# bioinfo-pf-curie/mpiBWA

Hardware: AMD Instinct MI355X
Metric: Mreads/s (whole node) 2x150 bp PE vs GRCh38-size reference; SAM bit-match (higher is better)
Workload: dtype int32

## Files before the change

mpibwa_amd/csrc/chain_kernel.hip:

```cpp
#include <hip/hip_runtime.h>
#include <hipcub/hipcub.hpp>
#include <cstdlib>
#include <mutex>
#include <utility>
#include <vector>
#include "hip_util.h"
#include "device.h"
#include "sortutil.h"

namespace mbw {

namespace {

typedef long long i64;

#define CK_MAXCH 9
#define CK_MAXCH_SMALL 4
#define CK_MAXSEEDS_SMALL 16
#define CK_MAXSEEDS 64
#define CK_MAXSEEDS_BIG 255
enum { F_POS_LO = 0, F_POS_HI, F_FIRST_Q, F_LAST_R_LO, F_LAST_R_HI, F_LAST_Q, F_LAST_LEN, F_RID, F_N, F_W, F_KEPT, F_FIRSTOV, F_NFIELDS };

template <int MAXCH>
struct StoreLds {
// ... 258 lines not shown
{
	extern __shared__ uint32_t lds_raw[];
	StoreLds<MAXCH> L;
	L.lane = threadIdx.x;
	L.tab = lds_raw;
	L.cid_ = (uint8_t *)(lds_raw + F_NFIELDS * MAXCH * 64);
	L.ord_ = L.cid_ + (MAXS + 1) * 64;
	L.tmp_ = L.ord_ + 16 * 64;
	int rd = blockIdx.x * 64 + threadIdx.x;
	if (list) { if (rd >= (int)*list_n) return; rd = list[rd]; }
	if (rd >= n_reads) return;
	const int ns = n_seeds[rd], lq = lens[rd];
	const int *gap = tab, *noflt = tab + 5 * tab_stride;
	if (LO >= 0) { if (n_chains[rd] != -1 || ns <= LO) return; }
	else if (ns == 0) { n_chains[rd] = 0; return; }
	if (ns > MAXS || !noflt[lq]) { n_chains[rd] = -1; return; }
	n_chains[rd] = chain_read(L, P, rd, ns, lq, seed_off[rd], l_rep, sa, qbl, ann_off, ann_alt, n_seqs, gap, chains, seeds, srt);
}

__global__ void __launch_bounds__(256)
chain_pick_kernel(int n_reads, const int *__restrict__ lens, const int *__restrict__ n_seeds, const int *__restrict__ n_chains,
                  const int *__restrict__ noflt, int lo, int hi, int cap, int *__restrict__ list, unsigned int *__restrict__ count)
{
	const int rd = blockIdx.x * 256 + threadIdx.x;
	const bool mine = rd < n_reads && n_chains[rd] == -1 && n_seeds[rd] > lo && n_seeds[rd] <= hi && noflt[lens[rd]] != 0;
	const unsigned long long m = __ballot(mine);
	if (!m) return;
	const int lane = threadIdx.x & 63, lead = __ffsll((long long)m) - 1;
	unsigned int base = 0;
	if (lane == lead) base = atomicAdd(count, (unsigned int)__popcll(m));
	base = __shfl(base, lead);
	const unsigned int at = base + (unsigned int)__popcll(m & ((1ull << lane) - 1));
	if (mine && at < (unsigned int)cap) list[at] = rd;
}

#define HV_NONE 0xFFFFu
__host__ __device__ constexpr size_t hv_lds_bytes(int cap) { return (size_t)(cap + 64) * 24; }
__host__ __device__ constexpr size_t hv_scratch_bytes(int cap) { return (size_t)cap * (4 + 7 * 2 + 8 + 4) + 512; }
struct HvStore {
	uint32_t *rid;
	uint16_t *head, *cid, *next, *ord;
	uint32_t *last_off;
	uint16_t *first_q, *last_q, *last_len, *tail, *nmem;
};
__device__ __forceinline__ bool hv_lt(uint32_t a, uint32_t b) { return (a >> 16) > (b >> 16); }
#define HV_FRAMES 32
__device__ __forceinline__ void hv_sort(uint32_t *a, int n)
{
	int fs[HV_FRAMES], ft[HV_FRAMES], fd[HV_FRAMES];
	ks_introsort_at(n, [a](int k) -> uint32_t & { return a[k]; }, KsFramesAt{fs, ft, fd}, hv_lt);
}
__device__ __forceinline__ void hv_sync()
{
	__builtin_amdgcn_fence(__ATOMIC_RELEASE, "wavefront");
	__builtin_amdgcn_wave_barrier();
	__builtin_amdgcn_fence(__ATOMIC_ACQUIRE, "wavefront");
}
__device__ __forceinline__ int hv_bcast(int v) { return __builtin_amdgcn_readfirstlane(v); }

template <int CAP>
__global__ void __launch_bounds__(64)
chain_heavy_kernel(ChainParams P, const int *__restrict__ list, const unsigned int *__restrict__ list_n, unsigned int *work, int list_cap,
                   const int *__restrict__ lens, const int *__restrict__ n_seeds, const int *__restrict__ l_rep, const i64 *__restrict__ seed_off,
                   const unsigned long long *__restrict__ sa, const int32_t *__restrict__ qbl, const i64 *__restrict__ ann_off,
                   const uint8_t *__restrict__ ann_alt, int n_seqs, const int *__restrict__ gap, uint8_t *__restrict__ scratch,
                   DevChain *__restrict__ chains, DevSeed *__restrict__ seeds, unsigned int *__restrict__ srt, int *__restrict__ n_chains)
// ... 339 lines not shown
	std::lock_guard<std::mutex> lk(side_mu);
	for (auto &e : sides) if (e.first == st) return e.second;
	ChainSide sd;
	for (int k = 0; k < 2; ++k) { HIP_OK(hipStreamCreateWithFlags(&sd.s[k], hipStreamNonBlocking)); HIP_OK(hipEventCreateWithFlags(&sd.join[k], hipEventDisableTiming)); }
	HIP_OK(hipEventCreateWithFlags(&sd.fork, hipEventDisableTiming));
	sides.emplace_back(st, sd);
	return sd;
}

void launch_chain(void *stream, const ChainParams &P, int n_reads, const int *d_len, const int *d_nseeds, const int *d_lrep,
                  const int64_t *d_seed_off, const uint64_t *d_sa, const int32_t *d_qbl, const int64_t *d_ann_off, const uint8_t *d_ann_alt,
                  int n_seqs, const int *d_tab, int tab_stride, DevChain *d_chains, DevSeed *d_seeds, unsigned int *d_srt, int *d_nchains,
                  void *d_scratch)
{
	if (n_reads <= 0) return;
	const size_t lds_s = chain_lds_bytes(CK_MAXSEEDS_SMALL, CK_MAXCH_SMALL), lds = chain_lds_bytes(CK_MAXSEEDS, CK_MAXCH), lds_big = chain_lds_bytes(CK_MAXSEEDS_BIG, CK_MAXCH);
	static bool s_attr = false;
	if (!s_attr) {
		if (lds > 64 * 1024) HIP_OK(hipFuncSetAttribute((const void *)chain_kernel<CK_MAXSEEDS, CK_MAXCH, 0>, hipFuncAttributeMaxDynamicSharedMemorySize, (int)lds));
		if (lds_big > 64 * 1024) HIP_OK(hipFuncSetAttribute((const void *)chain_kernel<CK_MAXSEEDS_BIG, CK_MAXCH, CK_MAXSEEDS>, hipFuncAttributeMaxDynamicSharedMemorySize, (int)lds_big));
		s_attr = true;
	}
	hipStream_t st = (hipStream_t)stream;
	const dim3 grid((n_reads + 63) / 64), block(64);
#define CHAIN_ARGS P, n_reads, d_len, d_nseeds, d_lrep, (const i64 *)d_seed_off, (const unsigned long long *)d_sa, d_qbl, (const i64 *)d_ann_off, d_ann_alt, n_seqs, d_tab, \
	               tab_stride, d_chains, d_seeds, d_srt, d_nchains
#define LAUNCH_HEAVY(CAP, waves, s, list, n, work, scr)                                                                                                       \
	hipLaunchKernelGGL((chain_heavy_kernel<CAP>), dim3(waves), dim3(64), hv_lds_bytes(CAP), s, P, (const int *)(list), (const unsigned int *)(n), work,      \
	                   n_reads, d_len, d_nseeds, d_lrep, (const i64 *)d_seed_off, (const unsigned long long *)d_sa, d_qbl, (const i64 *)d_ann_off, d_ann_alt, \
	                   n_seqs, d_tab, scr, d_chains, d_seeds, d_srt, d_nchains)
	const int big = getenv("MPIBWA_CHAIN_BIG") ? atoi(getenv("MPIBWA_CHAIN_BIG")) : 2;
	int *list_a = (int *)d_scratch, *list_b = list_a + n_reads;
	unsigned int *count = (unsigned int *)(list_b + n_reads);
	int *list_h1 = (int *)((uint8_t *)count + 512), *list_h2 = list_h1 + n_reads;
	uint8_t *scr_t = (uint8_t *)(((uintptr_t)(list_h2 + n_reads) + 255) & ~(uintptr_t)255);
	uint8_t *scr_s = scr_t + HV_WAVES_T * hv_scratch_bytes(256), *scr_l = scr_s + HV_WAVES_S * hv_scratch_bytes(1024);
	HIP_OK(hipMemsetAsync(count, 0, 64, st));
	auto pick = [&](int lo, int hi, int *list, unsigned int *n) {
		hipLaunchKernelGGL(chain_pick_kernel, dim3((n_reads + 255) / 256), dim3(256), 0, st, n_reads, d_len, d_nseeds, (const int *)d_nchains, d_tab + 5 * tab_stride, lo, hi,
		                   n_reads, list, n);
	};
	hipLaunchKernelGGL((chain_kernel<CK_MAXSEEDS_SMALL, CK_MAXCH_SMALL, -1>), grid, block, lds_s, st, CHAIN_ARGS, (const int *)nullptr, (const unsigned int *)nullptr);
	pick(0, CK_MAXSEEDS, list_a, count + 1);
	hipLaunchKernelGGL((chain_kernel<CK_MAXSEEDS, CK_MAXCH, 0>), grid, block, lds, st, CHAIN_ARGS, (const int *)list_a, (const unsigned int *)(count + 1));
	if (big >= 1) {
		pick(CK_MAXSEEDS, CK_MAXSEEDS_BIG, list_b, count + 2);
		hipLaunchKernelGGL((chain_kernel<CK_MAXSEEDS_BIG, CK_MAXCH, CK_MAXSEEDS>), grid, block, lds_big, st, CHAIN_ARGS, (const int *)list_b, (const unsigned int *)(count + 2));
	}
	if (big >= 2) {
		int *list_t = list_a;
		pick(0, CK_MAXSEEDS_BIG, list_t, count);
		const bool heavy = !(getenv("MPIBWA_CHAIN_HEAVY") && atoi(getenv("MPIBWA_CHAIN_HEAVY")) == 0);
		ChainSide sd = {};
		if (heavy) {
			static bool s_attr2 = false;
			if (!s_attr2) {
				HIP_OK(hipFuncSetAttribute((const void *)chain_heavy_kernel<4096>, hipFuncAttributeMaxDynamicSharedMemorySize, (int)hv_lds_bytes(4096)));
				s_attr2 = true;
			}
			pick(CK_MAXSEEDS_BIG, 1024, list_h1, count + 4);
			pick(1024, 4096, list_h2, count + 6);
			sd = chain_side_streams(st);
			HIP_OK(hipEventRecord(sd.fork, st));
			for (int k = 0; k < 2; ++k) HIP_OK(hipStreamWaitEvent(sd.s[k], sd.fork, 0));
			LAUNCH_HEAVY(4096, HV_WAVES_L, sd.s[0], list_h2, count + 6, count + 7, scr_l);
			LAUNCH_HEAVY(1024, HV_WAVES_S, sd.s[1], list_h1, count + 4, count + 5, scr_s);
		}
		LAUNCH_HEAVY(256, HV_WAVES_T, st, list_t, count, count + 3, scr_t);
		if (heavy)
			for (int k = 0; k < 2; ++k) { HIP_OK(hipEventRecord(sd.join[k], sd.s[k])); HIP_OK(hipStreamWaitEvent(st, sd.join[k], 0)); }
	}
#undef LAUNCH_HEAVY
#undef CHAIN_ARGS
	HIP_OK(hipGetLastError());
}

}
```

mpibwa_amd/csrc/phase1.hip:

```cpp
#include "pipeline.h"

namespace mbw {

static int c2a_early_mode() { const char *e = getenv("MPIBWA_C2A_EARLY"); return e ? atoi(e) : 1; }
static bool dev_dedup_on()
{
	const char *on = getenv("MPIBWA_DEV_DEDUP"), *off = getenv("MPIBWA_HOST_DEDUP");
	return on && atoi(on) != 0 && !(off && atoi(off) != 0);
}
class TurnLock {
public:
	void lock()
	{
		std::unique_lock<std::mutex> lk(m_);
		const unsigned long long mine = next_++;
		cv_.wait(lk, [&]() { return serving_ == mine; });
	}
	void unlock()
	{
		{ std::lock_guard<std::mutex> lk(m_); ++serving_; }
		cv_.notify_all();
	}
private:
	std::mutex m_;
	std::condition_variable cv_;
	unsigned long long next_ = 0, serving_ = 0;
};
static TurnLock g_smem_turn, g_c2a_turn;
static std::mutex g_pes_lock;

void Call::phase1(int lo, int hi, LaneBufs &L, HostBuf &reg_arena, hipStream_t lst, int lane_thr, P1 &ps)
{
	static const bool take_turns = !(getenv("MPIBWA_TURNS") && atoi(getenv("MPIBWA_TURNS")) == 0);
	const int n_sb = hi - lo;
	bseq1_t *seqs_r = seqs + lo;
	const int64_t *d_off_r = D.d_off + lo;
	const int *d_len_r = D.d_len + lo;
	const uint8_t *d_seq = D.d_seq;
	HIP_OK(hipSetDevice(ix.device));
	stage(2);
	parallel_for(lane_thr, n_sb, 4096, [&](int i) {
		char *s = seqs_r[i].seq;
		uint8_t *d = flat + off[lo + i];
		for (int k = 0; k < seqs_r[i].l_seq; ++k) {
			s[k] = s[k] < 4 ? s[k] : (char)nt4_table[(uint8_t)s[k]];
			d[k] = (uint8_t)s[k];
		}
	});
	HIP_OK(hipMemcpyAsync((uint8_t *)W.seq.p + off[lo], flat + off[lo], (size_t)(off[hi] - off[lo]) + (hi == n ? 16 : 0), hipMemcpyHostToDevice, lst));
	EvTimer ev_smem, ev_sa, ev_ext;
	unsigned long long *d_cnt = (unsigned long long *)L.cnt.ensure(256);
	unsigned long long *cnt = (unsigned long long *)L.h_cnt.ensure(256);
	const int TS = max_len + 2;
	std::vector<int> tab;
	c2a_length_tables(opt, max_len, tab);
	const int *gap_h = tab.data();
	int *d_tab = (int *)L.tab.ensure(tab.size() * 4);
	HIP_OK(hipMemcpyAsync(d_tab, tab.data(), tab.size() * 4, hipMemcpyHostToDevice, lst));

	double t1 = now_ms();
	uint64_t range_bases = 0;
	for (int i = 0; i < n_sb; ++i) range_bases += lens[lo + i];
	int cap = std::max(64, std::min(max_len, 96));
	uint64_t *d_intv; int *d_nintv;
	size_t per_quad = 0;
	int n_quads = smem_grid_quads(max_len, &per_quad);
	void *d_scr = L.scratch.ensure(per_quad * n_quads);
	int *d_nseeds = (int *)L.nseeds.ensure((size_t)n_sb * 4), *d_lrep = (int *)L.lrep.ensure((size_t)n_sb * 4);
	int *nseeds = (int *)L.h_nseeds.ensure((size_t)n_sb * 4 + 8), *lrep = (int *)L.h_lrep.ensure((size_t)n_sb * 4 + 8);
	int *nintv = (int *)L.h_nintv.ensure((size_t)n_sb * 4 + 8);
	const char *ce = getenv("MPIBWA_SMEM_COUNT");
	const bool count_blocks = ce && atoi(ce) != 0;
	for (;;) {
		d_intv = (uint64_t *)L.intv.ensure((size_t)n_sb * cap * 32);
		d_nintv = (int *)L.nintv.ensure((size_t)n_sb * 4);
		HIP_OK(hipMemsetAsync(d_cnt, 0, 256, lst));
		stage(20);
		std::unique_lock<TurnLock> turn(g_smem_turn, std::defer_lock);
		if (take_turns) turn.lock();
		stage(21);
		ev_smem.start(lst);
		launch_smem(lst, ix.fm, smem_params(opt), n_sb, d_seq, d_off_r, d_len_r, cap, d_intv, d_nintv, max_len, d_cnt, d_scr, per_quad, n_quads, count_blocks);
		ev_smem.stop(lst);
		launch_seed_prep(lst, n_sb, cap, d_intv, d_nintv, opt->max_occ, d_nseeds, d_lrep);
		HIP_OK(hipMemcpyAsync(cnt, d_cnt, 64, hipMemcpyDeviceToHost, lst));
		HIP_OK(hipMemcpyAsync(nseeds, d_nseeds, (size_t)n_sb * 4, hipMemcpyDeviceToHost, lst));
		HIP_OK(hipMemcpyAsync(lrep, d_lrep, (size_t)n_sb * 4, hipMemcpyDeviceToHost, lst));
		HIP_OK(hipMemcpyAsync(nintv, d_nintv, (size_t)n_sb * 4, hipMemcpyDeviceToHost, lst));
		stream_wait(lst);
		HIP_OK(hipGetLastError());
		if (take_turns) turn.unlock();
		ps.k_smem += ev_smem.ms();
		if (cnt[2] == 0) break;
		cap *= 4;
	}
	ps.smem_bytes = count_blocks ? cnt[1] * 64 + range_bases : 0;
	ps.smem_tab_bytes = cnt[4] * 64;
	double t2 = now_ms();
	stage(3);

	int64_t *seed_off = (int64_t *)L.h_seed_off.ensure((size_t)(n_sb + 1) * 8 + 64);
	seed_off[0] = 0;
	uint64_t n_intv = 0;
	for (int i = 0; i < n_sb; ++i) { seed_off[i + 1] = seed_off[i] + nseeds[i]; n_intv += nintv[i]; }
	const int64_t S = seed_off[n_sb];
	if (count_blocks) ps.smem_bytes += n_intv * 32;
	ps.n_intv = n_intv; ps.n_seeds = S;
	uint64_t *sa = (uint64_t *)L.h_sa.ensure((size_t)S * 8 + 8);
	int32_t *qbl = (int32_t *)L.h_qbl.ensure((size_t)S * 8 + 8);
	const bool host_chain_all = getenv("MPIBWA_HOST_CHAIN") != nullptr;
	const bool dev_chain = !host_chain_all && S > 0;
	int *nch = nullptr;
	DevChain *d_chains = nullptr; DevSeed *d_seeds = nullptr; unsigned int *d_srt = nullptr;
	if (S > 0) {
		int64_t *d_seed_off = (int64_t *)L.seed_off.ensure((size_t)(n_sb + 1) * 8);
		uint64_t *d_rows = (uint64_t *)L.rows.ensure((size_t)S * 8), *d_sa = (uint64_t *)L.sa.ensure((size_t)S * 8);
		int32_t *d_qbl = (int32_t *)L.qbl.ensure((size_t)S * 8);
		HIP_OK(hipMemcpyAsync(d_seed_off, seed_off, (size_t)(n_sb + 1) * 8, hipMemcpyHostToDevice, lst));
		launch_seed_enum(lst, n_sb, cap, d_intv, d_nintv, opt->max_occ, d_seed_off, d_rows, d_qbl);
		if (S > 0x7fffffff) die("too many seeds in one batch");
		HIP_OK(hipMemsetAsync(d_cnt, 0, 256, lst));
		ev_sa.start(lst);
		if (ix.fm.sa_full) launch_sa_dense(lst, ix.fm, (int)S, d_rows, d_sa);
		else launch_sa(lst, ix.fm, (int)S, d_rows, d_sa, d_cnt);
		ev_sa.stop(lst);
// ... 166 lines not shown
	const bool dev_dedup = dev_dedup_on();
	const uint8_t *dd_status = nullptr;
	const int *dd_m = nullptr, *dd_keep = nullptr;
	if (n_slots == 0) {
		memset(nregs, 0, (size_t)n_sb * 4);
		if (d_pr_nfirst) { HIP_OK(hipMemsetAsync(d_pr_nfirst + lo, 0, (size_t)n_sb * 4, lst)); stream_wait(lst); }
	} else {
		int *d_chain_beg = (int *)L.chain_off.ensure((size_t)n_sb * 4), *d_chain_cnt = (int *)L.chain_cnt.ensure((size_t)n_sb * 4);
		int *d_reg_beg = (int *)L.reg_off.ensure((size_t)n_sb * 4);
		d_chains = (DevChain *)L.chains.ensure((size_t)std::max<int64_t>(base + NC, 1) * sizeof(DevChain));
		d_seeds = (DevSeed *)L.seeds.ensure((size_t)n_slots * sizeof(DevSeed));
		d_srt = (unsigned int *)L.srt.ensure((size_t)n_slots * 4);
		DevReg *d_regs = (DevReg *)L.regs.ensure((size_t)n_slots * sizeof(DevReg));
		int *d_nregs = (int *)L.nregs.ensure((size_t)(n_sb + 1) * 4);
		HIP_OK(hipMemcpyAsync(d_chain_beg, chain_beg, (size_t)n_sb * 4, hipMemcpyHostToDevice, lst));
		HIP_OK(hipMemcpyAsync(d_chain_cnt, chain_cnt, (size_t)n_sb * 4, hipMemcpyHostToDevice, lst));
		HIP_OK(hipMemcpyAsync(d_reg_beg, reg_beg, (size_t)n_sb * 4, hipMemcpyHostToDevice, lst));
		if (NC) HIP_OK(hipMemcpyAsync(d_chains + base, hchains, (size_t)NC * sizeof(DevChain), hipMemcpyHostToDevice, lst));
		if (NS) HIP_OK(hipMemcpyAsync(d_seeds + base, hseeds, (size_t)NS * sizeof(DevSeed), hipMemcpyHostToDevice, lst));
		if (NS) HIP_OK(hipMemcpyAsync(d_srt + base, hsrt, (size_t)NS * 4, hipMemcpyHostToDevice, lst));
		unsigned long long *d_c2a_stat = (unsigned long long *)L.c2a_stat.ensure(C2A_STAT_SLOTS * 64);
		HIP_OK(hipMemsetAsync(d_c2a_stat, 0, C2A_STAT_SLOTS * 64, lst));
		int *order = (int *)L.h_order.ensure((size_t)n_sb * 4 + 8);
		c2a_launch_order(n_sb, nseeds, order);
		int *d_order = (int *)L.order.ensure((size_t)n_sb * 4);
		HIP_OK(hipMemcpyAsync(d_order, order, (size_t)n_sb * 4, hipMemcpyHostToDevice, lst));
		static const int heavy_t = getenv("MPIBWA_C2A_HEAVY") ? atoi(getenv("MPIBWA_C2A_HEAVY")) : 8;
		const C2aUnits units = c2a_prepare_units(lst, L.grp, heavy_t, n_sb, chain_cnt, (size_t)std::max<int64_t>(base + NC, 1), d_chain_beg, d_reg_beg,
		                                         d_chains, d_nregs, [](void *s) { stream_wait((hipStream_t)s); });
		C2aParams cp;
		ExtParams ep;
		c2a_params(opt, bns->l_pac, c2a_early_mode(), cp, ep);
		const int64_t guess = std::min<int64_t>(n_slots, (int64_t)2 * n_sb + 1024);
		uint8_t *d_dd_status = nullptr, *h_dd_status = nullptr;
		int *d_dd_m = nullptr, *d_dd_keep = nullptr, *d_dd_list = nullptr, *h_dd_m = nullptr, *h_dd_keep = nullptr;
		std::unique_ptr<EvTimer> ev_dd;
		if (dev_dedup) {
			ev_dd.reset(new EvTimer());
			d_dd_status = (uint8_t *)L.dd_status.ensure((size_t)n_sb);
			d_dd_m = (int *)L.dd_m.ensure((size_t)n_sb * 4);
			d_dd_keep = (int *)L.dd_keep.ensure((size_t)n_slots * 4);
			d_dd_list = (int *)L.dd_list.ensure(dedup_list_ints(n_sb) * 4);
			h_dd_status = (uint8_t *)L.h_dd_status.ensure((size_t)n_sb + 8);
			h_dd_m = (int *)L.h_dd_m.ensure((size_t)n_sb * 4 + 8);
			h_dd_keep = (int *)L.h_dd_keep.ensure((size_t)guess * 4 + 8);
		}
		stage(50);
		std::unique_lock<TurnLock> turn(g_c2a_turn, std::defer_lock);
		if (take_turns) turn.lock();
		stage(51);
		ev_ext.start(lst);
		launch_c2a(lst, cp, ep, n_sb, d_seq, d_off_r, d_len_r, d_chain_beg, d_chain_cnt, d_chains, d_seeds, d_srt, d_reg_beg, d_regs, d_nregs,
		           d_tab, TS, (const uint8_t *)ix.d_pac, d_c2a_stat, max_len, d_order, units.max_units > 0 ? &units : nullptr);
		ev_ext.stop(lst);
		int *d_reg_pos = (int *)L.reg_pos.ensure((size_t)(n_sb + 1) * 4);
		DevReg *d_packed = (DevReg *)L.regs_packed.ensure((size_t)n_slots * sizeof(DevReg));
		const size_t tmp_bytes = reg_pack_tmp_bytes(n_sb);
		void *d_tmp = L.pack_tmp.ensure(tmp_bytes);
		launch_reg_pack(lst, n_sb, d_reg_beg, d_nregs, d_reg_pos, d_regs, d_packed, d_tmp, tmp_bytes, units.max_units > 0 ? &units : nullptr, d_chain_beg, d_chain_cnt);
		if (d_pr_first) launch_first_reg(lst, n_sb, d_reg_pos, d_nregs, d_packed, d_pr_first + (size_t)lo * PR_MAXREG, d_pr_nfirst + lo);
		if (dev_dedup) {
			ev_dd->start(lst);
			launch_dedup(lst, dedup_params(opt, bns->l_pac), n_sb, d_packed, d_reg_pos, d_nregs, d_dd_status, d_dd_m, d_dd_keep, d_dd_list);
			ev_dd->stop(lst);
		}
		hregs = (DevReg *)L.h_regs.ensure((size_t)guess * sizeof(DevReg) + 8);
		unsigned long long *stat_h = (unsigned long long *)L.h_c2a_stat.ensure(C2A_STAT_SLOTS * 64);
		HIP_OK(hipMemcpyAsync(stat_h, d_c2a_stat, C2A_STAT_SLOTS * 64, hipMemcpyDeviceToHost, lst));
		HIP_OK(hipMemcpyAsync(nregs, d_nregs, (size_t)n_sb * 4, hipMemcpyDeviceToHost, lst));
		HIP_OK(hipMemcpyAsync(hregs, d_packed, (size_t)guess * sizeof(DevReg), hipMemcpyDeviceToHost, lst));
		if (dev_dedup) {
			HIP_OK(hipMemcpyAsync(h_dd_status, d_dd_status, (size_t)n_sb, hipMemcpyDeviceToHost, lst));
			HIP_OK(hipMemcpyAsync(h_dd_m, d_dd_m, (size_t)n_sb * 4, hipMemcpyDeviceToHost, lst));
			HIP_OK(hipMemcpyAsync(h_dd_keep, d_dd_keep, (size_t)guess * 4, hipMemcpyDeviceToHost, lst));
		}
		stream_wait(lst);
		HIP_OK(hipGetLastError());
		if (take_turns) turn.unlock();
		ps.k_ext = ev_ext.ms();
		for (int k = 0; k < 4; ++k) { cnt[k] = 0; for (int sl = 0; sl < C2A_STAT_SLOTS; ++sl) cnt[k] += stat_h[sl * 8 + k]; }
		ps.cells = cnt[0]; ps.n_ext = cnt[1];
		if (cp.early == 2 && cnt[3]) die("c2a_kernel: %llu of %llu extensions change when their row loops stop early", cnt[3], cnt[1]);
		if (getenv("MPIBWA_CPUSEC")) fprintf(stderr, "[c2a] %llu extensions, %llu without DP, %llu cells, kernel %.2f ms\n", cnt[1], cnt[2], cnt[0], ev_ext.ms());
		for (int i = 0; i < n_sb; ++i) reg_pos[i + 1] = reg_pos[i] + nregs[i];
		const int64_t NR = reg_pos[n_sb];
		if (NR > guess) {
			DevReg *all = (DevReg *)L.h_regs2.ensure((size_t)NR * sizeof(DevReg) + 8);
			HIP_OK(hipMemcpyAsync(all, d_packed, (size_t)NR * sizeof(DevReg), hipMemcpyDeviceToHost, lst));
			if (dev_dedup) {
				int *all_keep = (int *)L.h_dd_keep2.ensure((size_t)NR * 4 + 8);
				HIP_OK(hipMemcpyAsync(all_keep, d_dd_keep, (size_t)NR * 4, hipMemcpyDeviceToHost, lst));
				h_dd_keep = all_keep;
			}
			stream_wait(lst);
			hregs = all;
		}
		if (dev_dedup) {
			dd_status = h_dd_status; dd_m = h_dd_m; dd_keep = h_dd_keep;
			ps.k_dedup = ev_dd->ms();
			if (getenv("MPIBWA_CPUSEC")) {
				unsigned long long c[5] = {0, 0, 0, 0, 0};
				for (int i = 0; i < n_sb; ++i) ++c[dd_status[i] < 5 ? dd_status[i] : 0];
				fprintf(stderr, "[dedup] kernels %.2f ms; reads taken %llu, more than %d regions %llu, to patch %llu\n", ps.k_dedup, c[DD_TAKEN], DD_MAXREG,
				        c[DD_HOST_MAXREG], c[DD_HOST_PATCH]);
			}
		}
	}
	double t5 = now_ms();
	stage(6);

	const int SLACK = 4;
	std::vector<int64_t> slice(n_sb + 1);
	slice[0] = 0;
	for (int i = 0; i < n_sb; ++i) slice[i + 1] = slice[i] + nregs[i] + SLACK;
	HReg *arena = (HReg *)reg_arena.ensure((size_t)slice[n_sb] * sizeof(HReg));
	parallel_for(lane_thr, n_sb, 256, [&](int i) {
// ... 92 lines not shown
```

mpibwa_amd/csrc/pipeline.h:

```cpp
#ifndef MBW_PIPELINE_H
#define MBW_PIPELINE_H
#include <hip/hip_runtime.h>
#include <algorithm>
#include <atomic>
#include <memory>
#include <mutex>
#include <chrono>
#include <condition_variable>
#include <deque>
#include <cmath>
#include <cstdio>
#include <cstdlib>
#include <cstring>
#include <thread>
#include <vector>
#include <sys/resource.h>
#include <sys/time.h>
#include <unistd.h>

#include "hip_util.h"
#include "device.h"
#include "host.h"
#include "hprof.h"

// ... 111 lines not shown
		std::atomic<int> next{0};
		int n, nb, chunk;
		F *f;
		void work(int tid)
		{
			for (;;) {
				int b = next.fetch_add(1);
				if (b >= nb) break;
				(*f)(tid, b, b * chunk, std::min(n, (b + 1) * chunk));
			}
		}
	} R;
	R.n = n; R.nb = nb; R.chunk = chunk; R.f = &f;
	HelperPool &P = HelperPool::get();
	if (P.enabled() && n_threads > 1) {
		HelperPool::Job job;
		job.run = [](void *r, int tid) { ((Region *)r)->work(tid); };
		job.region = &R;
		P.run(n_threads - 1, job, [](void *r) { ((Region *)r)->work(0); }, &R);
		return;
	}
	std::vector<std::thread> th;
	for (int t = 1; t < n_threads; ++t) th.emplace_back([&R, t]() { R.work(t); });
	R.work(0);
	for (auto &t : th) t.join();
}

double now_ms();
double sys_sec();
long page_faults();
double cpu_sec();
void stage(int id);
void stream_wait(hipStream_t st);

struct EvTimer {
	hipEvent_t a, b;
	EvTimer() { HIP_OK(hipEventCreate(&a)); HIP_OK(hipEventCreate(&b)); }
	~EvTimer() { (void)hipEventDestroy(a); (void)hipEventDestroy(b); }
	void start(hipStream_t s) { HIP_OK(hipEventRecord(a, s)); }
	void stop(hipStream_t s) { HIP_OK(hipEventRecord(b, s)); }
	double ms() { HIP_OK(hipEventSynchronize(b)); float m = 0; HIP_OK(hipEventElapsedTime(&m, a, b)); return m; }
};

struct HostBuf {
	void *p = nullptr; size_t cap = 0;
	void *ensure(size_t bytes) { if (bytes > cap) { free(p); cap = bytes + bytes / 4 + 4096; p = malloc(cap); if (!p) die("out of memory"); } return p; }
};

struct LaneBufs {
	PinBuf h_nch, h_cbeg, h_ccnt, h_rbeg, h_nseeds, h_lrep, h_nintv, h_cnt, h_seed_off, h_c2a_stat, h_order;
	PinBuf h_sa, h_qbl, h_chains, h_seeds, h_srt, h_regs, h_regs2, h_nregs;
	DevBuf nch, chain_cnt, reg_pos, regs_packed, pack_tmp, order, chain_scratch, c2a_stat;
	C2aGroupBufs grp;
	DevBuf intv, nintv, cnt, scratch, nseeds, lrep, seed_off, rows, qbl, sa;
	DevBuf chain_off, chains, seeds, srt, reg_off, regs, nregs, tab;
	DevBuf dd_status, dd_m, dd_keep, dd_list;
	PinBuf h_dd_status, h_dd_m, h_dd_keep, h_dd_keep2;
};
struct JobBufs {
	DevBuf req, hdr, pool, cnt, lists, base, arena, used, ooff, olen;
	PinBuf h_hdr, h_pool, h_base, h_arena, h_ooff, h_olen;
};
struct ChunkBufs {
	PinBuf h_off, h_len, h_flat;
	DevBuf seq, off, len, ann_off, ann_alt, agap;
	DevBuf sdesc, squal, snames, snoff, sann_names, sann_noff;
	PinBuf h_sdesc, h_names, h_noff, h_qual;
	DevBuf pr_first, pr_nfirst, pr_ok, pr_status, pr_ptab, pr_req, pr_desc;
	PinBuf h_pr_ok, h_pr_status, h_pr_tab;
	PinBuf h_mreq[2], h_mres[2], h_mlist[2];
	DevBuf mreq[2], mres[2], mrows[2], mlist[2], mtail[2];
	PinBuf h_wwork[2], h_wlists[2], h_wloff[2], h_wmfirst[2], h_wtags[2], h_wtoff[2], h_wstatus[2];
	DevBuf wwork[2], wlists[2], wloff[2], wmfirst[2], wtags[2], wtoff[2], wstatus[2], wreq[2], wdesc[2];
	JobBufs wave_job[2];
	PinBuf h_wxcnt[2], h_wxdst[2];
	DevBuf wxreq[2], wxcnt[2], wxdst[2], xa_req[2], xa_desc;
	JobBufs xa_job[2];
	PinBuf h_areq[2];
	JobBufs host_job[2];
	JobBufs dev_job[2];
	PinBuf h_small[2];
};
static const int MAX_LANES = 4;
static const int MAX_CALLS = 12;
struct CallCtx {
	std::vector<DevBuf *> bufs;
	struct Open { Open(std::vector<DevBuf *> *l) { g_devbuf_owner = l; } } open_{&bufs};
	LaneBufs ws[MAX_LANES];
	HostBuf reg_arena[17];
	ChunkBufs gws;
	hipStream_t p_streams[MAX_LANES] = {nullptr}, a_streams[2] = {nullptr, nullptr}, d_streams[2] = {nullptr, nullptr};
	bool busy = false;
	const bseq1_t *seq_lo = nullptr, *seq_hi = nullptr;
	int calls_done = 0;
	struct Close { Close() { g_devbuf_owner = nullptr; } } close_;
	size_t device_bytes() const { size_t b = 0; for (const DevBuf *d : bufs) b += d->cap; return b; }
	void release_device() { for (DevBuf *d : bufs) d->release(); calls_done = 0; }
};

struct P1 { double k_smem = 0, k_sa = 0, k_ext = 0, k_dedup = 0, smem = 0, sa = 0, chain = 0, ext = 0, regs = 0; uint64_t smem_bytes = 0, smem_tab_bytes = 0, sa_bytes = 0, cells = 0, n_ext = 0, n_intv = 0, n_seeds = 0, n_chains = 0, n_dedup_dev = 0, n_dedup_host = 0; };

struct Job {
	JobBufs *B = nullptr;
	bool launched = false, sam_launched = false;
	hipStream_t st = 0;
	size_t n_req = 0, pool_bytes = 0, arena_bytes = 0;
	int n_reads = 0;
	AlnHdr *d_hdr = nullptr; uint8_t *d_pool = nullptr; unsigned long long *d_cnt = nullptr;
	unsigned long long *small_cnt = nullptr, *small_used = nullptr;
	EvTimer ev;
	const AlnHdrH *hdr = nullptr; const uint8_t *pool = nullptr;
	const uint8_t *sarena = nullptr; const unsigned long long *sooff = nullptr; const int *solen = nullptr;
};
struct Part {
	int lo = 0, hi = 0, slot = 0;
	AlnReqH *req = nullptr;
	size_t n_req = 0;
	std::vector<uint32_t> base;
	Job host;
	Job dev;
	MswReqH *mreq = nullptr; MswResH *mres = nullptr;
	std::vector<uint32_t> mbase;
	size_t n_mreq = 0;
	hipStream_t mst = 0;
	EvTimer mev;
	bool m_launched = false, msw_launched = false;
	std::vector<int> work;
	std::vector<unsigned> w_mfirst;
	std::vector<int> w_toff;
	std::vector<int16_t> w_tags;
	const uint8_t *wstatus = nullptr;
	int n_wave_dec = 0;
	Job wave;
// ... 101 lines not shown
```

mpibwa_amd/csrc/pipeline.hip:

```cpp
#include "pipeline.h"

namespace mbw {

static mi355x_stats_t g_stats;

static int usable_cpus_now()
{
	int hw = (int)std::thread::hardware_concurrency();
	if (hw <= 0) hw = 1;
	if (FILE *fp = fopen("/sys/fs/cgroup/cpu.max", "r")) {
		char q[64];
		long long period = 0;
		if (fscanf(fp, "%63s %lld", q, &period) == 2 && strcmp(q, "max") != 0 && period > 0) {
			long long quota = atoll(q);
			int c = (int)((quota + period - 1) / period);
			if (c >= 1 && c < hw) hw = c;
		}
		fclose(fp);
	}
	return hw;
}
int usable_cpus() { static const int c = usable_cpus_now(); return c; }

static int env_int(const char *const *names, int dflt)
// ... 62 lines not shown
	{
		while (!stop.load()) {
			int nw = 0, nh = 0, st[SAMPLE_SLOTS], ns = 0;
			for (int i = 0; i < SAMPLE_SLOTS; ++i) {
				const int v = g_stage[i].load(std::memory_order_relaxed);
				if (!v) continue;
				st[ns++] = v;
				const int id = v & 63, w = (v & STG_WAIT) != 0;
				if (w) ++nw; else if (id != 20 && id != 50) ++nh;
			}
			if (ns >= min_calls) {
				++n_samples; ++by_wait[nw]; ++by_host[nh];
				for (int k = 0; k < ns; ++k) ++in_stage[st[k] & 63][(st[k] & STG_WAIT) != 0];
				if (!nw) { ++n_gpu_idle; for (int k = 0; k < ns; ++k) ++host_when_idle[st[k] & 63]; }
				if (!nh) ++n_host_idle;
			}
			usleep(250);
		}
	}
	void report()
	{
		if (!n_samples) return;
		fprintf(stderr, "[sample] %llu samples with a call in flight; no call waiting for the GPU in %.1f %%, no call on the host in %.1f %%\n",
		        (unsigned long long)n_samples, 100.0 * n_gpu_idle / n_samples, 100.0 * n_host_idle / n_samples);
		fprintf(stderr, "[sample] calls waiting for the GPU:");
		for (int k = 0; k <= 12; ++k) fprintf(stderr, " %d:%.1f%%", k, 100.0 * by_wait[k] / n_samples);
		fprintf(stderr, "\n[sample] calls working on the host:");
		for (int k = 0; k <= 12; ++k) fprintf(stderr, " %d:%.1f%%", k, 100.0 * by_host[k] / n_samples);
		fprintf(stderr, "\n[sample] stage: mean calls in it on the host / waiting for the GPU / on the host while no call waits for the GPU\n");
		for (int id = 0; id < SAMPLE_STAGES; ++id)
			if (in_stage[id][0] + in_stage[id][1])
				fprintf(stderr, "[sample]   %2d: %.3f %.3f %.3f\n", id, (double)in_stage[id][0] / n_samples, (double)in_stage[id][1] / n_samples,
				        n_gpu_idle ? (double)host_when_idle[id] / n_gpu_idle : 0.0);
	}
};
static StageSampler *g_sampler = nullptr;
void sampler_report()
{
	if (!g_sampler) return;
	g_sampler->stop.store(true);
	g_sampler->th.join();
	g_sampler->report();
	delete g_sampler;
	g_sampler = nullptr;
}

void stream_wait(hipStream_t st)
{
	static const bool spin = getenv("MPIBWA_SPIN_WAIT") != nullptr;
	struct Mark {
		Mark() { if (t_stage) t_stage->fetch_or(STG_WAIT, std::memory_order_relaxed); }
		~Mark() { if (t_stage) t_stage->fetch_and(~STG_WAIT, std::memory_order_relaxed); }
	} mark;
	if (!spin) {
		for (;;) {
			hipError_t e = hipStreamQuery(st);
			if (e == hipSuccess) break;
			if (e != hipErrorNotReady) HIP_OK(e);
			(void)hipGetLastError();
			usleep(60);
		}
	}
	HIP_OK(hipStreamSynchronize(st));
}


void Call::pack()
{
	stage(29);
	off = (int64_t *)W.h_off.ensure((size_t)(n + 1) * 8 + 64);
	lens = (int *)W.h_len.ensure((size_t)n * 4 + 64);
	{
		const int BLK = 8192, nb = (n + BLK - 1) / BLK;
		std::vector<int64_t> bsum(nb + 1, 0);
		std::vector<int> bmax(nb, 0);
		parallel_for(n_thr, nb, 1, [&](int b) {
			const int lo = b * BLK, hi = std::min(n, lo + BLK);
			int64_t sl = 0;
			int m = 0;
			for (int i = lo; i < hi; ++i) {
				const int l = seqs[i].l_seq;
				lens[i] = l; sl += (l + 15) & ~15; m = std::max(m, l);
			}
			bsum[b + 1] = sl; bmax[b] = m;
		});
		for (int b = 0; b < nb; ++b) { bsum[b + 1] += bsum[b]; max_len = std::max(max_len, bmax[b]); }
		parallel_for(n_thr, nb, 1, [&](int b) {
			const int lo = b * BLK, hi = std::min(n, lo + BLK);
			int64_t o = bsum[b];
			for (int i = lo; i < hi; ++i) { off[i] = o; o += (lens[i] + 15) & ~15; }
		});
		off[n] = bsum[nb];
	}
	stage(30);
	flat_bytes = (size_t)off[n] + 16;
	flat = (uint8_t *)W.h_flat.ensure(flat_bytes);
// ... 322 lines not shown
```

Baseline: 6.847.

## Release GPU turn locks after kernel finishes instead of after copy-back

The seeding and extension turn locks now release once the main kernel's stop event completes, so the follow-on prep kernels, packing and device-to-host copies run outside the serialized section and the next caller can launch sooner. The turn lock is rewritten as a ticket lock with a configurable admission width, and turn queue, hold and tail clocks are recorded for diagnostics. Some buffer allocations are hoisted out of the locked region. An opt-in, size-ordered bucketing of heavy chain read lists is also added. Releasing earlier lets calls overlap on the GPU, at the cost of contention between a call's tail work and the next call's kernel.

```diff
diff --git a/mpibwa_amd/csrc/chain_kernel.hip b/mpibwa_amd/csrc/chain_kernel.hip
--- a/mpibwa_amd/csrc/chain_kernel.hip
+++ b/mpibwa_amd/csrc/chain_kernel.hip
@@ -314,6 +314,42 @@
 	base = __shfl(base, lead);
 	const unsigned int at = base + (unsigned int)__popcll(m & ((1ull << lane) - 1));
 	if (mine && at < (unsigned int)cap) list[at] = rd;
+}
+
+#define HV_BUCKETS 8
+__device__ __forceinline__ int hv_list_bucket(int ns, int &bucket, int buckets)
+{
+	if (ns <= CK_MAXSEEDS_BIG || ns > 4096) return -1;
+	const int l = ns > 1024, lo = l ? 1024 : CK_MAXSEEDS_BIG, hi = l ? 4096 : 1024;
+	bucket = buckets - 1 - (int)((long long)(ns - lo - 1) * buckets / (hi - lo));
+	return l;
+}
+__global__ void __launch_bounds__(256)
+chain_bucket_count_kernel(int n_reads, const int *__restrict__ lens, const int *__restrict__ n_seeds, const int *__restrict__ n_chains,
+                          const int *__restrict__ noflt, int buckets, unsigned int *__restrict__ cnt, unsigned int *__restrict__ n1, unsigned int *__restrict__ n2)
+{
+	const int rd = blockIdx.x * 256 + threadIdx.x;
+	if (rd >= n_reads || n_chains[rd] != -1 || noflt[lens[rd]] == 0) return;
+	int b = 0;
+	const int l = hv_list_bucket(n_seeds[rd], b, buckets);
+	if (l < 0) return;
+	atomicAdd(cnt + l * HV_BUCKETS + b, 1u);
+	atomicAdd(l ? n2 : n1, 1u);
+}
+__global__ void __launch_bounds__(256)
+chain_bucket_place_kernel(int n_reads, const int *__restrict__ lens, const int *__restrict__ n_seeds, const int *__restrict__ n_chains,
+                          const int *__restrict__ noflt, int buckets, const unsigned int *__restrict__ cnt, unsigned int *__restrict__ fill,
+                          int *__restrict__ list1, int *__restrict__ list2)
+{
+	const int rd = blockIdx.x * 256 + threadIdx.x;
+	if (rd >= n_reads || n_chains[rd] != -1 || noflt[lens[rd]] == 0) return;
+	int b = 0;
+	const int l = hv_list_bucket(n_seeds[rd], b, buckets);
+	if (l < 0) return;
+	unsigned int at = 0;
+	for (int k = 0; k < b; ++k) at += cnt[l * HV_BUCKETS + k];
+	at += atomicAdd(fill + l * HV_BUCKETS + b, 1u);
+	if (at < (unsigned int)n_reads) (l ? list2 : list1)[at] = rd;
 }
 
 #define HV_NONE 0xFFFFu
@@ -719,10 +755,11 @@
 	const int big = getenv("MPIBWA_CHAIN_BIG") ? atoi(getenv("MPIBWA_CHAIN_BIG")) : 2;
 	int *list_a = (int *)d_scratch, *list_b = list_a + n_reads;
 	unsigned int *count = (unsigned int *)(list_b + n_reads);
+	unsigned int *bucket_cnt = count + 16, *bucket_fill = bucket_cnt + 2 * HV_BUCKETS;
 	int *list_h1 = (int *)((uint8_t *)count + 512), *list_h2 = list_h1 + n_reads;
 	uint8_t *scr_t = (uint8_t *)(((uintptr_t)(list_h2 + n_reads) + 255) & ~(uintptr_t)255);
 	uint8_t *scr_s = scr_t + HV_WAVES_T * hv_scratch_bytes(256), *scr_l = scr_s + HV_WAVES_S * hv_scratch_bytes(1024);
-	HIP_OK(hipMemsetAsync(count, 0, 64, st));
+	HIP_OK(hipMemsetAsync(count, 0, (16 + 4 * HV_BUCKETS) * 4, st));
 	auto pick = [&](int lo, int hi, int *list, unsigned int *n) {
 		hipLaunchKernelGGL(chain_pick_kernel, dim3((n_reads + 255) / 256), dim3(256), 0, st, n_reads, d_len, d_nseeds, (const int *)d_nchains, d_tab + 5 * tab_stride, lo, hi,
 		                   n_reads, list, n);
@@ -745,8 +782,17 @@
 				HIP_OK(hipFuncSetAttribute((const void *)chain_heavy_kernel<4096>, hipFuncAttributeMaxDynamicSharedMemorySize, (int)hv_lds_bytes(4096)));
 				s_attr2 = true;
 			}
-			pick(CK_MAXSEEDS_BIG, 1024, list_h1, count + 4);
-			pick(1024, 4096, list_h2, count + 6);
+			const bool ordered = getenv("MPIBWA_CHAIN_ORDER") && atoi(getenv("MPIBWA_CHAIN_ORDER")) != 0;
+			const int buckets = HV_BUCKETS;
+			if (!ordered) {
+				pick(CK_MAXSEEDS_BIG, 1024, list_h1, count + 4);
+				pick(1024, 4096, list_h2, count + 6);
+			} else {
+			hipLaunchKernelGGL(chain_bucket_count_kernel, dim3((n_reads + 255) / 256), dim3(256), 0, st, n_reads, d_len, d_nseeds, (const int *)d_nchains, d_tab + 5 * tab_stride,
+			                   buckets, bucket_cnt, count + 4, count + 6);
+			hipLaunchKernelGGL(chain_bucket_place_kernel, dim3((n_reads + 255) / 256), dim3(256), 0, st, n_reads, d_len, d_nseeds, (const int *)d_nchains, d_tab + 5 * tab_stride,
+			                   buckets, (const unsigned int *)bucket_cnt, bucket_fill, list_h1, list_h2);
+			}
 			sd = chain_side_streams(st);
 			HIP_OK(hipEventRecord(sd.fork, st));
 			for (int k = 0; k < 2; ++k) HIP_OK(hipStreamWaitEvent(sd.s[k], sd.fork, 0));
diff --git a/mpibwa_amd/csrc/phase1.hip b/mpibwa_amd/csrc/phase1.hip
--- a/mpibwa_amd/csrc/phase1.hip
+++ b/mpibwa_amd/csrc/phase1.hip
@@ -1,4 +1,5 @@
 #include "pipeline.h"
+#include "turn_lock.h"
 
 namespace mbw {
 
@@ -8,30 +9,30 @@
 	const char *on = getenv("MPIBWA_DEV_DEDUP"), *off = getenv("MPIBWA_HOST_DEDUP");
 	return on && atoi(on) != 0 && !(off && atoi(off) != 0);
 }
-class TurnLock {
-public:
-	void lock()
-	{
-		std::unique_lock<std::mutex> lk(m_);
-		const unsigned long long mine = next_++;
-		cv_.wait(lk, [&]() { return serving_ == mine; });
-	}
-	void unlock()
-	{
-		{ std::lock_guard<std::mutex> lk(m_); ++serving_; }
-		cv_.notify_all();
-	}
-private:
-	std::mutex m_;
-	std::condition_variable cv_;
-	unsigned long long next_ = 0, serving_ = 0;
+static bool take_turns_on() { const char *e = getenv("MPIBWA_TURNS"); return !(e && atoi(e) == 0); }
+static bool tail_in_turn_on() { const char *e = getenv("MPIBWA_TURN_TAIL"); return e && atoi(e) != 0; }
+static const int TURN_WIDTH_SMEM = 1, TURN_WIDTH_C2A = 1;
+static void turn_widths(int &w_smem, int &w_c2a)
+{
+	w_smem = TURN_WIDTH_SMEM; w_c2a = TURN_WIDTH_C2A;
+	const char *e = getenv("MPIBWA_TURN_WIDTH");
+	if (!e || !*e) return;
+	w_smem = w_c2a = std::max(1, atoi(e));
+	if (const char *c = strchr(e, ',')) w_c2a = std::max(1, atoi(c + 1));
+}
+struct Event {
+	hipEvent_t e;
+	Event() { HIP_OK(hipEventCreate(&e)); }
+	~Event() { (void)hipEventDestroy(e); }
 };
 static TurnLock g_smem_turn, g_c2a_turn;
 static std::mutex g_pes_lock;
 
 void Call::phase1(int lo, int hi, LaneBufs &L, HostBuf &reg_arena, hipStream_t lst, int lane_thr, P1 &ps)
 {
-	static const bool take_turns = !(getenv("MPIBWA_TURNS") && atoi(getenv("MPIBWA_TURNS")) == 0);
+	const bool take_turns = take_turns_on(), tail_in_turn = tail_in_turn_on();
+	int w_smem = 1, w_c2a = 1;
+	turn_widths(w_smem, w_c2a);
 	const int n_sb = hi - lo;
 	bseq1_t *seqs_r = seqs + lo;
 	const int64_t *d_off_r = D.d_off + lo;
@@ -49,6 +50,7 @@
 	});
 	HIP_OK(hipMemcpyAsync((uint8_t *)W.seq.p + off[lo], flat + off[lo], (size_t)(off[hi] - off[lo]) + (hi == n ? 16 : 0), hipMemcpyHostToDevice, lst));
 	EvTimer ev_smem, ev_sa, ev_ext;
+	Event ev_tail;
 	unsigned long long *d_cnt = (unsigned long long *)L.cnt.ensure(256);
 	unsigned long long *cnt = (unsigned long long *)L.h_cnt.ensure(256);
 	const int TS = max_len + 2;
@@ -76,21 +78,29 @@
 		d_nintv = (int *)L.nintv.ensure((size_t)n_sb * 4);
 		HIP_OK(hipMemsetAsync(d_cnt, 0, 256, lst));
 		stage(20);
-		std::unique_lock<TurnLock> turn(g_smem_turn, std::defer_lock);
-		if (take_turns) turn.lock();
+		const double q0 = now_ms();
+		TurnHold turn(g_smem_turn, take_turns, w_smem);
+		const double q1 = now_ms();
+		double q2 = q1;
 		stage(21);
 		ev_smem.start(lst);
 		launch_smem(lst, ix.fm, smem_params(opt), n_sb, d_seq, d_off_r, d_len_r, cap, d_intv, d_nintv, max_len, d_cnt, d_scr, per_quad, n_quads, count_blocks);
 		ev_smem.stop(lst);
+		if (!tail_in_turn) { event_wait(ev_smem.b); HIP_OK(hipGetLastError()); turn.release(); q2 = now_ms(); stage(26); }
 		launch_seed_prep(lst, n_sb, cap, d_intv, d_nintv, opt->max_occ, d_nseeds, d_lrep);
 		HIP_OK(hipMemcpyAsync(cnt, d_cnt, 64, hipMemcpyDeviceToHost, lst));
 		HIP_OK(hipMemcpyAsync(nseeds, d_nseeds, (size_t)n_sb * 4, hipMemcpyDeviceToHost, lst));
 		HIP_OK(hipMemcpyAsync(lrep, d_lrep, (size_t)n_sb * 4, hipMemcpyDeviceToHost, lst));
 		HIP_OK(hipMemcpyAsync(nintv, d_nintv, (size_t)n_sb * 4, hipMemcpyDeviceToHost, lst));
+		HIP_OK(hipEventRecord(ev_tail.e, lst));
 		stream_wait(lst);
 		HIP_OK(hipGetLastError());
-		if (take_turns) turn.unlock();
-		ps.k_smem += ev_smem.ms();
+		if (tail_in_turn) { turn.release(); q2 = now_ms(); }
+		const double k_ms = ev_smem.ms();
+		float tail_ms = 0;
+		HIP_OK(hipEventElapsedTime(&tail_ms, ev_smem.b, ev_tail.e));
+		ps.k_smem += k_ms;
+		ps.tc_smem.queue += q1 - q0; ps.tc_smem.hold += q2 - q1; ps.tc_smem.kernel += k_ms; ps.tc_smem.tail += tail_ms; ++ps.tc_smem.n;
 		if (cnt[2] == 0) break;
 		cap *= 4;
 	}
@@ -323,6 +333,12 @@
 		ExtParams ep;
 		c2a_params(opt, bns->l_pac, c2a_early_mode(), cp, ep);
 		const int64_t guess = std::min<int64_t>(n_slots, (int64_t)2 * n_sb + 1024);
+		int *d_reg_pos = (int *)L.reg_pos.ensure((size_t)(n_sb + 1) * 4);
+		DevReg *d_packed = (DevReg *)L.regs_packed.ensure((size_t)n_slots * sizeof(DevReg));
+		const size_t tmp_bytes = reg_pack_tmp_bytes(n_sb);
+		void *d_tmp = L.pack_tmp.ensure(tmp_bytes);
+		hregs = (DevReg *)L.h_regs.ensure((size_t)guess * sizeof(DevReg) + 8);
+		unsigned long long *stat_h = (unsigned long long *)L.h_c2a_stat.ensure(C2A_STAT_SLOTS * 64);
 		uint8_t *d_dd_status = nullptr, *h_dd_status = nullptr;
 		int *d_dd_m = nullptr, *d_dd_keep = nullptr, *d_dd_list = nullptr, *h_dd_m = nullptr, *h_dd_keep = nullptr;
 		std::unique_ptr<EvTimer> ev_dd;
@@ -337,17 +353,16 @@
 			h_dd_keep = (int *)L.h_dd_keep.ensure((size_t)guess * 4 + 8);
 		}
 		stage(50);
-		std::unique_lock<TurnLock> turn(g_c2a_turn, std::defer_lock);
-		if (take_turns) turn.lock();
+		const double q0 = now_ms();
+		TurnHold turn(g_c2a_turn, take_turns, w_c2a);
+		const double q1 = now_ms();
+		double q2 = q1;
 		stage(51);
 		ev_ext.start(lst);
 		launch_c2a(lst, cp, ep, n_sb, d_seq, d_off_r, d_len_r, d_chain_beg, d_chain_cnt, d_chains, d_seeds, d_srt, d_reg_beg, d_regs, d_nregs,
 		           d_tab, TS, (const uint8_t *)ix.d_pac, d_c2a_stat, max_len, d_order, units.max_units > 0 ? &units : nullptr);
 		ev_ext.stop(lst);
-		int *d_reg_pos = (int *)L.reg_pos.ensure((size_t)(n_sb + 1) * 4);
-		DevReg *d_packed = (DevReg *)L.regs_packed.ensure((size_t)n_slots * sizeof(DevReg));
-		const size_t tmp_bytes = reg_pack_tmp_bytes(n_sb);
-		void *d_tmp = L.pack_tmp.ensure(tmp_bytes);
+		if (!tail_in_turn) { event_wait(ev_ext.b); HIP_OK(hipGetLastError()); turn.release(); q2 = now_ms(); stage(52); }
 		launch_reg_pack(lst, n_sb, d_reg_beg, d_nregs, d_reg_pos, d_regs, d_packed, d_tmp, tmp_bytes, units.max_units > 0 ? &units : nullptr, d_chain_beg, d_chain_cnt);
 		if (d_pr_first) launch_first_reg(lst, n_sb, d_reg_pos, d_nregs, d_packed, d_pr_first + (size_t)lo * PR_MAXREG, d_pr_nfirst + lo);
 		if (dev_dedup) {
@@ -355,8 +370,6 @@
 			launch_dedup(lst, dedup_params(opt, bns->l_pac), n_sb, d_packed, d_reg_pos, d_nregs, d_dd_status, d_dd_m, d_dd_keep, d_dd_list);
 			ev_dd->stop(lst);
 		}
-		hregs = (DevReg *)L.h_regs.ensure((size_t)guess * sizeof(DevReg) + 8);
-		unsigned long long *stat_h = (unsigned long long *)L.h_c2a_stat.ensure(C2A_STAT_SLOTS * 64);
 		HIP_OK(hipMemcpyAsync(stat_h, d_c2a_stat, C2A_STAT_SLOTS * 64, hipMemcpyDeviceToHost, lst));
 		HIP_OK(hipMemcpyAsync(nregs, d_nregs, (size_t)n_sb * 4, hipMemcpyDeviceToHost, lst));
 		HIP_OK(hipMemcpyAsync(hregs, d_packed, (size_t)guess * sizeof(DevReg), hipMemcpyDeviceToHost, lst));
@@ -365,14 +378,23 @@
 			HIP_OK(hipMemcpyAsync(h_dd_m, d_dd_m, (size_t)n_sb * 4, hipMemcpyDeviceToHost, lst));
 			HIP_OK(hipMemcpyAsync(h_dd_keep, d_dd_keep, (size_t)guess * 4, hipMemcpyDeviceToHost, lst));
 		}
+		HIP_OK(hipEventRecord(ev_tail.e, lst));
 		stream_wait(lst);
 		HIP_OK(hipGetLastError());
-		if (take_turns) turn.unlock();
+		if (tail_in_turn) { turn.release(); q2 = now_ms(); }
 		ps.k_ext = ev_ext.ms();
+		float tail_ms = 0;
+		HIP_OK(hipEventElapsedTime(&tail_ms, ev_ext.b, ev_tail.e));
+		ps.tc_c2a.queue = q1 - q0; ps.tc_c2a.hold = q2 - q1; ps.tc_c2a.kernel = ps.k_ext; ps.tc_c2a.tail = tail_ms; ps.tc_c2a.n = 1;
 		for (int k = 0; k < 4; ++k) { cnt[k] = 0; for (int sl = 0; sl < C2A_STAT_SLOTS; ++sl) cnt[k] += stat_h[sl * 8 + k]; }
 		ps.cells = cnt[0]; ps.n_ext = cnt[1];
 		if (cp.early == 2 && cnt[3]) die("c2a_kernel: %llu of %llu extensions change when their row loops stop early", cnt[3], cnt[1]);
 		if (getenv("MPIBWA_CPUSEC")) fprintf(stderr, "[c2a] %llu extensions, %llu without DP, %llu cells, kernel %.2f ms\n", cnt[1], cnt[2], cnt[0], ev_ext.ms());
+		if (getenv("MPIBWA_CPUSEC") || getenv("MPIBWA_TURN_CLOCKS")) {
+			const TurnClock &a = ps.tc_smem, &b = ps.tc_c2a;
+			fprintf(stderr, "[turn] seeding: %d holds, queued %.2f ms, held %.2f ms (kernel %.2f), tail %.2f ms; extension: queued %.2f ms, held %.2f ms (kernel %.2f), tail %.2f ms\n",
+			        a.n, a.queue, a.hold, a.kernel, a.tail, b.queue, b.hold, b.kernel, b.tail);
+		}
 		for (int i = 0; i < n_sb; ++i) reg_pos[i + 1] = reg_pos[i] + nregs[i];
 		const int64_t NR = reg_pos[n_sb];
 		if (NR > guess) {
diff --git a/mpibwa_amd/csrc/pipeline.h b/mpibwa_amd/csrc/pipeline.h
--- a/mpibwa_amd/csrc/pipeline.h
+++ b/mpibwa_amd/csrc/pipeline.h
@@ -167,6 +167,7 @@
 double cpu_sec();
 void stage(int id);
 void stream_wait(hipStream_t st);
+void event_wait(hipEvent_t ev);
 
 struct EvTimer {
 	hipEvent_t a, b;
@@ -233,7 +234,8 @@
 	void release_device() { for (DevBuf *d : bufs) d->release(); calls_done = 0; }
 };
 
-struct P1 { double k_smem = 0, k_sa = 0, k_ext = 0, k_dedup = 0, smem = 0, sa = 0, chain = 0, ext = 0, regs = 0; uint64_t smem_bytes = 0, smem_tab_bytes = 0, sa_bytes = 0, cells = 0, n_ext = 0, n_intv = 0, n_seeds = 0, n_chains = 0, n_dedup_dev = 0, n_dedup_host = 0; };
+struct TurnClock { double queue = 0, hold = 0, kernel = 0, tail = 0; int n = 0; };
+struct P1 { TurnClock tc_smem, tc_c2a; double k_smem = 0, k_sa = 0, k_ext = 0, k_dedup = 0, smem = 0, sa = 0, chain = 0, ext = 0, regs = 0; uint64_t smem_bytes = 0, smem_tab_bytes = 0, sa_bytes = 0, cells = 0, n_ext = 0, n_intv = 0, n_seeds = 0, n_chains = 0, n_dedup_dev = 0, n_dedup_host = 0; };
 
 struct Job {
 	JobBufs *B = nullptr;
diff --git a/mpibwa_amd/csrc/pipeline.hip b/mpibwa_amd/csrc/pipeline.hip
--- a/mpibwa_amd/csrc/pipeline.hip
+++ b/mpibwa_amd/csrc/pipeline.hip
@@ -118,6 +118,8 @@
 			if (in_stage[id][0] + in_stage[id][1])
 				fprintf(stderr, "[sample]   %2d: %.3f %.3f %.3f\n", id, (double)in_stage[id][0] / n_samples, (double)in_stage[id][1] / n_samples,
 				        n_gpu_idle ? (double)host_when_idle[id] / n_gpu_idle : 0.0);
+		auto in_st = [&](int id) { return (double)(in_stage[id][0] + in_stage[id][1]) / n_samples; };
+		fprintf(stderr, "[sample] turns: seeding %.3f queueing, %.3f holding; extension %.3f queueing, %.3f holding\n", in_st(20), in_st(21), in_st(50), in_st(51));
 	}
 };
 static StageSampler *g_sampler = nullptr;
@@ -148,6 +150,25 @@
 		}
 	}
 	HIP_OK(hipStreamSynchronize(st));
+}
+
+void event_wait(hipEvent_t ev)
+{
+	static const bool spin = getenv("MPIBWA_SPIN_WAIT") != nullptr;
+	struct Mark {
+		Mark() { if (t_stage) t_stage->fetch_or(STG_WAIT, std::memory_order_relaxed); }
+		~Mark() { if (t_stage) t_stage->fetch_and(~STG_WAIT, std::memory_order_relaxed); }
+	} mark;
+	if (!spin) {
+		for (;;) {
+			hipError_t e = hipEventQuery(ev);
+			if (e == hipSuccess) break;
+			if (e != hipErrorNotReady) HIP_OK(e);
+			(void)hipGetLastError();
+			usleep(60);
+		}
+	}
+	HIP_OK(hipEventSynchronize(ev));
 }
 
 
diff --git a/mpibwa_amd/csrc/turn_lock.h b/mpibwa_amd/csrc/turn_lock.h
--- /dev/null
+++ b/mpibwa_amd/csrc/turn_lock.h
@@ -0,0 +1,53 @@
+#pragma once
+#include <condition_variable>
+#include <mutex>
+
+namespace mbw {
+
+class TurnLock {
+public:
+	template <class OnTicket, class OnAdmit>
+	void lock(int width, OnTicket on_ticket, OnAdmit on_admit)
+	{
+		if (width < 1) width = 1;
+		std::unique_lock<std::mutex> lk(m_);
+		const unsigned long long mine = next_++;
+		on_ticket(mine);
+		cv_[mine % SLOTS].wait(lk, [&]() { return admitted_ == mine && admitted_ - released_ < (unsigned long long)width; });
+		++admitted_;
+		on_admit(mine);
+		std::condition_variable &head = cv_[admitted_ % SLOTS];
+		lk.unlock();
+		head.notify_all();
+	}
+	void lock(int width = 1) { lock(width, [](unsigned long long) {}, [](unsigned long long) {}); }
+	void unlock()
+	{
+		std::condition_variable *head;
+		{ std::lock_guard<std::mutex> lk(m_); ++released_; head = &cv_[admitted_ % SLOTS]; }
+		head->notify_all();
+	}
+	unsigned long long queued()
+	{
+		std::lock_guard<std::mutex> lk(m_);
+		return next_ - admitted_;
+	}
+private:
+	std::mutex m_;
+	static const int SLOTS = 32;
+	std::condition_variable cv_[SLOTS];
+	unsigned long long next_ = 0, admitted_ = 0, released_ = 0;
+};
+
+class TurnHold {
+public:
+	TurnHold(TurnLock &t, bool on, int width) : t_(on ? &t : nullptr) { if (t_) t_->lock(width); }
+	~TurnHold() { release(); }
+	void release() { if (t_) { t_->unlock(); t_ = nullptr; } }
+	TurnHold(const TurnHold &) = delete;
+	TurnHold &operator=(const TurnHold &) = delete;
+private:
+	TurnLock *t_;
+};
+
+}
```

After: 6.877 (median of 3 runs). About the same (+0.4%).
